# meiqua/6DPose

Hardware: AMD Instinct MI355X
Metric: templates*Mpixels matched/sec on 640x480 RGB-D (higher is better)
Workload: dtype u8

## Files before the change

6dpose_amd/csrc/detector.cpp:

```cpp
#include <math.h>
#include <stdarg.h>
#include <stdio.h>
#include <stdlib.h>
#include <string.h>

#include <algorithm>
#include <system_error>
#include <chrono>
#include <memory>
#include <string>
#include <vector>
#include <map>

#include "detector_internal.h"
#include <sched.h>
#include <ctype.h>
#include "render_internal.h"

static thread_local std::string g_err;
int lm_set_error(int code, const char* fmt, ...) {
    char buf[1024];
    va_list ap;
    va_start(ap, fmt);
    vsnprintf(buf, sizeof(buf), fmt, ap);
// ... 147 lines not shown
    if (d->mstream) (void)hipStreamSynchronize(d->mstream);
    d->frame_rgb.release(); d->frame_depth.release(); d->nrm_raw.release();
    for (int i = 0; i < lm_detector::kSlots; ++i) {
        if (d->ingest.pinned[i]) (void)hipHostFree(d->ingest.pinned[i]);
        d->ingest.d_rgb[i].release();
        if (d->ingest.t0[i]) (void)hipEventDestroy(d->ingest.t0[i]);
        if (d->ingest.t1[i]) (void)hipEventDestroy(d->ingest.t1[i]);
    }
    if (d->ingest.stream) (void)hipStreamDestroy(d->ingest.stream);
    for (int a = 0; a < lm_detector::kSlots; ++a) { d->lm_arena[a].release(); d->sm_arena[a].release(); }
    for (int a = 0; a < lm_detector::kSlots; ++a) { d->bits_arena[a].release(); d->cbits_arena[a].release(); }
    for (auto& b : d->slot_rgb) b.release();
    for (auto& b : d->slot_depth) b.release();
    for (auto& l : d->lvl) { l.rgb.release(); l.mag.release(); l.ang.release(); l.nrm.release(); l.mask[0].release(); l.mask[1].release(); }
    d->d_entries.release(); d->d_feat_off.release(); d->d_feat_xy.release(); d->d_feat_word.release(); d->d_run_mask.release(); d->d_work.release();
    d->d_cands.release(); d->d_counters.release(); d->d_final.release(); d->d_matches_dev.release(); d->d_hash.release(); d->d_distinct_keys.release(); d->d_tiles.release(); d->d_todo.release(); d->d_work_cls.release(); d->d_work_tid.release();
    for (int l = 0; l < kMaxLevels; ++l) { d->train.mask[l].release(); d->train.lab[l].release(); d->train.hrun[l].release(); }
    d->train.user_mask.release();
    d->train.keys.release(); d->train.counts.release(); d->train.bbox.release(); d->train.out.release();
    for (auto& sl : d->slot) {
        if (sl.h_matches) (void)hipHostFree(sl.h_matches);
        if (sl.h_distinct) (void)hipHostFree(sl.h_distinct);
        if (sl.h_counters) (void)hipHostFree(sl.h_counters);
        if (sl.fe_done) (void)hipEventDestroy(sl.fe_done);
        for (auto& e : sl.ev) if (e) (void)hipEventDestroy(e);
        if (sl.done) (void)hipEventDestroy(sl.done);
    }
    if (d->xchg.stream) (void)hipStreamSynchronize(d->xchg.stream);
    for (int a = 0; a < lm_detector::kSlots; ++a) {
        d->xchg.d_merged[a].release();
        d->xchg.d_runs.release();
// ... 1174 lines not shown
}
static bool cbits_active(const lm_detector* d, int num_work) {
    return bits_active(d, num_work) && knobs().coarse_bits && d->coarse_mode == 0 && d->cbits_max_nf <= 16383;
}
static int frame_slot(lm_detector* d, int si, bool tiled, uint32_t tile_cap, FrameSlot* out) {
    lm_detector::Slot& sl = d->slot[si];
    const uint32_t cc = d->buf_cand_cap;
    FrameSlot F{};
    F.lm_arena = d->lm_arena[si].p; F.sm_arena = d->sm_arena[si].p;
    F.cands = d->d_cands.p + (size_t)cc * si;
    F.tiles = tiled ? d->d_tiles.p + (size_t)tile_cap * si : nullptr;
    F.todo = tiled ? d->d_todo.p + (size_t)cc * si : nullptr;
    F.counters = d->d_counters.p + (size_t)kCounterWords * si;
    F.matches_dev = d->d_matches_dev.p + (size_t)cc * si;
    F.dedupe_table = d->d_hash.p + dedupe_table_slots(cc) * (size_t)si;
    F.distinct_keys = d->d_distinct_keys.p + (size_t)cc * si;
    F.final_dev = d->d_final.p + 8 * (size_t)si;
    F.matches = nullptr;
    HIP_TRY(hipHostGetDevicePointer((void**)&F.distinct, sl.h_distinct, 0));
    HIP_TRY(hipHostGetDevicePointer((void**)&F.final_host, sl.h_counters, 0));
    *out = F;
    return LM_OK;
}

static int slot_begin(lm_detector* d, float threshold, const char* const* class_ids, int num_class_ids, const uint8_t* rgb, const uint16_t* depth,
                      const bool have_mask[2], int ring) {
    if (d->n_submitted - d->n_collected >= (uint64_t)lm_detector::kSlots)
        return lm_set_error(LM_ERR_INVALID, "%d frames already in flight: call lm_detector_collect first", lm_detector::kSlots);
    HIP_TRY(hipSetDevice(d->device));
    int rc;
// ... 6 lines not shown
        if (class_ids && num_class_ids > 0)
            for (int i = 0; i < num_class_ids; ++i) key.push_back(class_ids[i] ? class_ids[i] : "");
        const bool same = d->work_valid && key == d->work_key && d->work_key_rank == d->shard_rank && d->work_key_world == d->shard_world;
        if (d->pend_n && (!same || threshold != d->pend_threshold) && (rc = lm_launch_pending(d))) return rc;
    }
    if ((rc = build_work(d, class_ids, num_class_ids))) return rc;
    const int num_work = (int)d->work_pyr.size();
    const int K = lm_detector::kSlots;
    if (d->buf_cand_cap < d->cand_cap) {
        if ((rc = lm_launch_pending(d))) return rc;
        if ((rc = sync_all_streams(d))) return rc;
        const uint32_t cc = d->cand_cap;
        if ((rc = d->d_cands.ensure((size_t)cc * K))) return rc;
        if ((rc = d->d_matches_dev.ensure((size_t)cc * K))) return rc;
        if ((rc = d->d_hash.ensure(dedupe_table_slots(cc) * K))) return rc;
        if ((rc = d->d_distinct_keys.ensure((size_t)cc * K))) return rc;
        d->buf_cand_cap = cc;
    }
    if (!d->d_counters.p) {
        if ((rc = d->d_counters.ensure((size_t)kCounterWords * K))) return rc;
        if ((rc = d->d_final.ensure(8 * (size_t)K))) return rc;
        HIP_TRY(hipMemset(d->d_counters.p, 0, (size_t)kCounterWords * K * sizeof(unsigned long long)));
        HIP_TRY(hipMemset(d->d_final.p, 0, 8 * (size_t)K * sizeof(unsigned long long)));
    }
    const bool tiled = (tiles_wanted(d) && num_work > 0 && tile_plan_possible(d->geom)) || bits_active(d, num_work);
    const uint32_t tile_cap = d->buf_cand_cap / 2;
    if (tiled && (d->d_tiles.cap < (size_t)tile_cap * K || d->d_todo.cap < (size_t)d->buf_cand_cap * K)) {
        if ((rc = lm_launch_pending(d))) return rc;
        if ((rc = sync_all_streams(d))) return rc;
        if ((rc = d->d_tiles.ensure((size_t)tile_cap * K))) return rc;
// ... 72 lines not shown
    FrameBatch fb{};
    fb.nb = nb;
    int rc;
    for (int b = 0; b < nb; ++b)
        if ((rc = frame_slot(d, (first + b) % lm_detector::kSlots, tiled, tile_cap, &fb.f[b]))) return rc;
    hipStream_t ms = d->mstream, s = ms;
    for (int b = nb - 1; b >= 0; --b) {
        const int ring = d->slot[(first + b) % lm_detector::kSlots].ring;
        if (ring < 0) continue;
        if (hipEventQuery(d->ingest.t1[ring]) != hipSuccess) { (void)hipGetLastError(); HIP_TRY(hipStreamWaitEvent(s, d->ingest.t1[ring], 0)); }
        break;
    }
    if ((rc = order_after_default_stream(d, s))) return rc;
    HIP_TRY(hipEventRecord(lead.ev[0], s));
    const bool cbits = cbits_active(d, num_work);
    bool direct_low = knobs().fe_bits && d->fe_direct && bits && d->bits_all_in, direct_top = knobs().fe_bits && d->fe_direct && cbits;
    for (int l = 0; l + 1 < d->geom.levels; ++l) direct_low = direct_low && fe_bits_rows_possible(d->geom.lv[l].W, d->geom.lv[l].T);
    const LevelGeom& topl = d->geom.lv[d->geom.levels - 1];
    const uint32_t top_bit0[2] = {topl.lm_off[0] - d->cbits_byte0, topl.lm_off[1] - d->cbits_byte0};
    const bool top_ored = direct_top && fe_top_bits_kind(topl.W, topl.H, topl.T, top_bit0, d->fe_top_mode) == kFeTopBits;
    if (top_ored)
        for (int b = 0; b < nb; ++b) {
            const int si = (first + b) % lm_detector::kSlots;
            if (!d->cbits_clean[si]) HIP_TRY(hipMemsetAsync(d->cbits_arena[si].p, 0, (size_t)d->cbits_npairs * 8, s));
            d->cbits_clean[si] = false;
        }
#ifdef LM_DIAG
    static double lp_t[6]; static long lp_n;
    auto lp_now = [] { return std::chrono::duration<double>(std::chrono::steady_clock::now().time_since_epoch()).count(); };
    const double lp0 = host_seconds(tp_launch0), lp1 = lp_now();
// ... 28 lines not shown
    bool resident_in = false;
    for (int b = 0; b < nb; ++b) resident_in = resident_in || d->slot[(first + b) % lm_detector::kSlots].ring < 0;
    HIP_TRY(hipEventRecord(lead.ev[1], s));
    if (resident_in) HIP_TRY(hipEventRecord(lead.fe_done, s));
    for (int b = 0; b < nb; ++b)
        if (d->slot[(first + b) % lm_detector::kSlots].ring < 0) d->resident_reader = lead.fe_done;
    for (int b = 0; b < nb; ++b) {
        const lm_detector::Slot& sl = d->slot[(first + b) % lm_detector::kSlots];
        if (sl.ring < 0 && d->ingest.stream)
            for (int r = 0; r < lm_detector::kSlots; ++r)
                if (d->ingest.d_rgb[r].p && sl.in_rgb == d->ingest.d_rgb[r].p) d->ingest.reader[r] = lead.fe_done;
    }
    const uint32_t cap = std::min<uint32_t>(lead.match_cap, d->buf_cand_cap);
    auto enqueue_coarse = [&](hipStream_t st) -> int {
        { LM_CLOCK("launch_coarse");
        if (cbits) launch_coarse_bits(fb, tb, d->geom, d->d_entries.p, d->d_feat_off.p, d->d_work.p, num_work, threshold, d->buf_cand_cap, d->cbits_byte0, d->cbits_max_nf, st);
        else launch_coarse(fb, d->geom, d->d_entries.p, d->d_feat_off.p, d->d_work.p, num_work, threshold, d->buf_cand_cap, tile_cap, st);
        }
        HIP_TRY(hipEventRecord(lead.ev[3], st));
        return LM_OK;
    };
    auto enqueue_match = [&]() -> int {
        if (bits) {
            { LM_CLOCK("launch_local_bits");
            launch_local_bits(fb, bb, d->geom, d->d_entries.p, d->d_feat_word.p, d->d_work.p, d->buf_cand_cap, threshold, cap,
                              (uint32_t)dedupe_table_slots(d->buf_cand_cap), bits_grid(d, nb), d->bits_max_nf, ms); }
            if (bb.top_clear_units)
                for (int b = 0; b < nb; ++b)
                    if (bb.top_clear[b]) d->cbits_clean[(first + b) % lm_detector::kSlots] = true;
            if (!d->bits_all_in)
                launch_local(fb_rest, d->geom, d->d_entries.p, d->d_feat_off.p, d->d_feat_word.p, d->d_run_mask.p, d->d_feat_xy.p, d->d_work.p, d->buf_cand_cap, threshold, cap,
                             (uint32_t)dedupe_table_slots(d->buf_cand_cap), tile_cap, d->num_cus * 2, ms);
        } else
        if (num_work > 0)
            launch_local(fb, d->geom, d->d_entries.p, d->d_feat_off.p, d->d_feat_word.p, d->d_run_mask.p, d->d_feat_xy.p, d->d_work.p, d->buf_cand_cap, threshold, cap,
                         (uint32_t)dedupe_table_slots(d->buf_cand_cap), tile_cap, local_grid(d, nb), ms);
        HIP_TRY(hipEventRecord(lead.ev[4], ms));
        return LM_OK;
    };
    const int dedupe_blocks = knobs().dedupe_blocks > 0 ? knobs().dedupe_blocks
                                                        : std::max(64, std::min(d->num_cus * 2, (int)((d->ncand_hint + 255) / 256)));
    auto enqueue_dedupe = [&](hipStream_t st) -> int {
        if (num_work > 0) {
            LM_CLOCK("launch_dedupe");
            launch_dedupe(fb, d->buf_cand_cap, dedupe_table_slots(d->buf_cand_cap), d->d_work_cls.p, d->d_work_tid.p, dedupe_blocks, st);
        }
        else
            for (int b = 0; b < nb; ++b) HIP_TRY(hipMemsetAsync(fb.f[b].final_dev, 0, 8 * sizeof(unsigned long long), st));
        return LM_OK;
    };
    {
#ifdef LM_DIAG
        const double lp3 = lp_now();
#endif
        if ((rc = enqueue_coarse(ms))) return rc;
#ifdef LM_DIAG
        const double lp4 = lp_now();
// ... 293 lines not shown
    lm_timings tm{};
    tm.h2d_ms = sl.h2d_ms; tm.templates = sl.num_work; tm.coarse_bytes = sl.coarse_bytes;
    if (d->ingest.used[slot_index]) {
        d->ingest.used[slot_index] = false;
        float h = 0.f;
        if (hipEventElapsedTime(&h, d->ingest.t0[slot_index], d->ingest.t1[slot_index]) == hipSuccess) tm.h2d_ms = h;
    }
    const uint64_t evals = sl.num_work > 0 ? hc[5] : 0, lbytes = sl.num_work > 0 ? hc[6] : 0;
    uint64_t nm = 0;
    const Candidate* hm = sl.h_matches;
    if (sl.num_work > 0 && ncand > 0 && (sort_unique == 0 || sort_unique == 3 || d->reference_order))
        HIP_TRY(hipMemcpy(sl.h_matches, sl.matches_dev, (size_t)ncand * sizeof(Candidate), hipMemcpyDeviceToHost));
    if (sl.num_work == 0) nm = 0;
    else if (sort_unique == 0) { for (uint64_t i = 0; i < ncand; ++i) nm += hm[i].work >= 0; }
    else nm = hc[2];
    tm.coarse_candidates = (int64_t)ncand;
    d->ncand_hint = (uint64_t)ncand;
    tm.local_evals = (int64_t)evals;
    tm.local_bytes = (int64_t)lbytes;
    tm.matches_pre_unique = (int64_t)nm;
    tm.d2h_ms = 0.f;
    tm.batch_frames = sl.batch_n;
    if (hipEventElapsedTime(&tm.frontend_ms, lead.ev[0], lead.ev[1]) != hipSuccess ||
        hipEventElapsedTime(&tm.coarse_ms, lead.ev[1], lead.ev[3]) != hipSuccess ||
        hipEventElapsedTime(&tm.local_ms, lead.ev[3], lead.ev[4]) != hipSuccess ||
        hipEventElapsedTime(&tm.total_ms, lead.ev[0], lead.ev[4]) != hipSuccess) {
        (void)hipGetLastError();
        tm.frontend_ms = tm.coarse_ms = tm.local_ms = tm.d2h_ms = tm.total_ms = 0.f;
    }
    if (sort_unique < 0) {
// ... 231 lines not shown
    d->fe_direct = on != 0;
    d->fe_keep_top = (on & 2) != 0;
    d->fe_top_mode = (on & 4) ? 1 : ((on & 8) ? 2 : 0);
    return LM_OK;
}

extern "C" int lm_detector_get_paths(const lm_detector* d, int* refine, int* coarse) {
    if (!d || !refine || !coarse) return lm_set_error(LM_ERR_INVALID, "null argument");
    if (d->bank_dirty) return lm_set_error(LM_ERR_INVALID, "no match yet: the paths follow from the bank and the frame geometry");
    const bool bits = bits_active(d, 1);
    *refine = bits ? 0 : (d->geom.levels >= 2 && tiles_wanted(d) && tile_plan_possible(d->geom) ? 1 : 2);
    *coarse = cbits_active(d, 1) ? 0 : 1;
    return LM_OK;
}

extern "C" int lm_detector_flush(lm_detector* d) {
    if (!d) return lm_set_error(LM_ERR_INVALID, "null detector");
    return lm_launch_pending(d);
}

extern "C" int lm_detector_set_batch(lm_detector* d, int frames) {
    if (!d) return lm_set_error(LM_ERR_INVALID, "null detector");
    if (frames < 1 || frames > kMaxBatch) return lm_set_error(LM_ERR_INVALID, "frames per launch must be in [1, %d]", kMaxBatch);
    int rc = lm_launch_pending(d);
    if (rc) return rc;
    d->batch_max = frames;
    return LM_OK;
}

extern "C" int lm_detector_get_batch(const lm_detector* d) { return d ? d->batch_max : 0; }
// ... 98 lines not shown
```

6dpose_amd/csrc/detector_internal.h:

```cpp
#pragma once
#include <atomic>
#include <chrono>
#include <condition_variable>
#include <deque>
#include <functional>
#include <memory>
#include <mutex>
#include <string>
#include <thread>
#include <vector>

#include "../../include/amd_linemod.h"
#include "host_templates.h"
#include "knobs.h"
#include "lm_kernels.h"

int lm_set_error(int code, const char* fmt, ...);

#define HIP_TRY(expr)                                                                                         \
    do {                                                                                                      \
        hipError_t _e = (expr);                                                                               \
        if (_e != hipSuccess) return lm_set_error(LM_ERR_HIP, "%s failed: %s (%s:%d)", #expr, hipGetErrorString(_e), \
                                                  __FILE__, __LINE__);                                        \
    } while (0)
// ... 72 lines not shown
    std::vector<TemplEntry> h_entries;
    DevBuf<TemplEntry> d_entries;
    DevBuf<int32_t> d_feat_off;
    DevBuf<uint32_t> d_feat_xy;
    DevBuf<uint32_t> d_feat_word, d_run_mask;
    std::vector<int32_t> work_pyr;
    std::shared_ptr<std::vector<int32_t>> work_cls, work_tid;
    DevBuf<int32_t> d_work;
    std::vector<std::string> work_key;
    int work_key_rank = -1, work_key_world = -1;
    bool work_valid = false;
    int64_t work_coarse_bytes = 0;
    DevBuf<Candidate> d_cands;
    DevBuf<Candidate> d_matches_dev;
    DevBuf<unsigned long long> d_hash;
    DevBuf<TileRec> d_tiles;
    DevBuf<uint8_t> d_todo;
    bool use_tiles = true;
    bool reference_order = false;
    DevBuf<ulonglong2> d_distinct_keys;
    DevBuf<int32_t> d_work_cls, d_work_tid;
    DevBuf<unsigned long long> d_counters;
    DevBuf<unsigned long long> d_final;
    uint32_t cand_cap = 1u << 18;
    uint32_t buf_cand_cap = 0;
    struct Slot {
        Candidate* h_matches = nullptr;
        Candidate* h_distinct = nullptr;
        uint32_t match_cap = 0;
        unsigned long long* h_counters = nullptr;
// ... 130 lines not shown
```

6dpose_amd/csrc/knobs.h:

```cpp
#pragma once
#include <stdlib.h>

#ifndef LM_FE_WAVES
#define LM_FE_WAVES 7
#endif
constexpr int kFeWaves = LM_FE_WAVES;

namespace lm {

struct Knobs {
    int coarse_group = 4;
    int local_blocks = 0;
    int frame_batch = 0;
    int coarse_bits = 1;
    int bitplanes = 1;
    int fe_bits = 1;
    int fe_bits_split = 0;
    int first_batch = 3;
    int fe_rows_cs = 0;
    int nt_copy = 1;
    int dedupe_blocks = 0;
    int fe_wgs_per_cu = kFeWaves;
    int launch_slack_us = 0;
    int batch_queue = 0;
    int knn_blocks = 0;
    int icp_splits = 0;
    int icp_team = 0;
    int icp_builds = 0;
    int icp_team_min_points = 128;
    int icp_cut_index = 3;
    int icp_relaunch = 1;
    int icp_wide_sort = 1;
    int icp_maxshift = 3;
    int icp_maxshift_late = 4;
#ifdef LM_DIAG
    int coarse_dbg = 0;
// ... 6 lines not shown
    static const Knobs k = [] {
        Knobs v;
        auto geti = [](const char* name, int dflt) { const char* e = getenv(name); return e && e[0] ? atoi(e) : dflt; };
        v.coarse_group = geti("LM_COARSE_GROUP", v.coarse_group);
        v.local_blocks = geti("LM_LOCAL_BLOCKS", 0);
        v.frame_batch = geti("LM_FRAME_BATCH", 0);
        v.batch_queue = geti("LM_BATCH_QUEUE", 0);
        v.launch_slack_us = geti("LM_LAUNCH_SLACK_US", 0);
        v.fe_wgs_per_cu = geti("LM_FE_WGS_PER_CU", kFeWaves);
        v.bitplanes = geti("LM_BITPLANES", 1);
        v.coarse_bits = geti("LM_COARSE_BITS", 1);
        v.fe_bits = geti("LM_FE_BITS", 1);
        v.fe_bits_split = geti("LM_FE_BITS_SPLIT", 0);
        v.first_batch = geti("LM_FIRST_BATCH", v.first_batch);
        v.dedupe_blocks = geti("LM_DEDUPE_BLOCKS", 0);
        v.nt_copy = geti("LM_NT_COPY", 1);
        v.fe_rows_cs = geti("LM_FE_ROWS_CS", 0);
        v.knn_blocks = geti("LM_KNN_BLOCKS", 0);
        v.icp_splits = geti("LM_ICP_SPLITS", 0);
        v.icp_team = geti("LM_ICP_TEAM", 0);
        v.icp_builds = geti("LM_ICP_BUILDS", 0);
        v.icp_wide_sort = geti("LM_ICP_WIDE_SORT", 1);
        v.icp_relaunch = geti("LM_ICP_RELAUNCH", 1);
        v.icp_cut_index = geti("LM_ICP_CUT_INDEX", 3);
        v.icp_team_min_points = geti("LM_ICP_TEAM_MIN_POINTS", 128);
        if (v.icp_team_min_points < 1) v.icp_team_min_points = 1;
        v.icp_maxshift = geti("LM_ICP_MAXSHIFT", v.icp_maxshift);
        v.icp_maxshift_late = geti("LM_ICP_MAXSHIFT_LATE", v.icp_maxshift_late);
#ifdef LM_DIAG
        v.coarse_dbg = geti("LM_COARSE_DBG", 0);
// ... 10 lines not shown
```

6dpose_amd/csrc/lm_kernels.h:

```cpp
#pragma once
#include <hip/hip_runtime.h>
#include <stdint.h>

namespace lm {

void upload_normal_lut(const uint8_t lut400[400]);
void launch_color_quant(const uint8_t* rgb, float* mag, uint8_t* onehot, int W, int H, float thr_sq, hipStream_t s);
void launch_normals_fused(const uint16_t* depth, uint8_t* raw, uint8_t* med, int W, int H, int dist_thr, int diff_thr, hipStream_t s);
void launch_pyrdown_rgb(const uint8_t* src, uint8_t* dst, int W, int H, hipStream_t s);
void launch_nn_down2(const uint8_t* src, uint8_t* dst, int W, int H, hipStream_t s);
void launch_build_lm(const uint8_t* const quant[2], const uint8_t* const mask[2], uint8_t* const lm[2], uint8_t* const strips[2],
                     int W, int H, int T, hipStream_t s);

struct LmJob { const uint8_t* quant; const uint8_t* mask; uint8_t* lm; uint8_t* strips; };
enum { kFeNone = 0, kFeColour, kFeNormals, kFePyrDown, kFeNnDown, kFeBuildLm, kFeBitsRows, kFeTopBits, kFeTopBitsAligned, kFeTopBitsTile, kFeBitsRowsTile };
struct FeJob {
    int kind, gx, gy, gz, first;
    const void* in; void* out0; void* out1;
    int W, H, a, b;
    float f;
    uint32_t m_gx, m_gxgy, m_wd, m_t, m_np;
    int Wd, Hd;
    LmJob lm[2];
};
// ... 51 lines not shown
constexpr int kCandBits = 40;
constexpr unsigned long long kCandMask = (1ull << kCandBits) - 1ull;
constexpr int kMaxBatch = 8;
constexpr int kCounterWords = 64;
constexpr int kStatShards = 16;
struct FrameSlot {
    const uint8_t* lm_arena;
    const uint8_t* sm_arena;
    Candidate* cands;
    TileRec* tiles;
    uint8_t* todo;
    unsigned long long* counters;
    Candidate* matches;
    Candidate* matches_dev;
    unsigned long long* dedupe_table;
    Candidate* distinct;
    ulonglong2* distinct_keys;
    unsigned long long* final_dev;
    unsigned long long* final_host;
};
struct FrameBatch {
    int nb;
    int pad;
    FrameSlot f[kMaxBatch];
};

struct BitsBatch { const uint8_t* strips[kMaxBatch]; uint8_t* bits[kMaxBatch];
                   uint8_t* top_clear[kMaxBatch]; uint32_t top_clear_units; };
constexpr int kBitsSmallMax = 511;
void launch_pack_bits(const BitsBatch& B, int nb, const LevelGeom& lv, hipStream_t s);
void launch_local_bits(const FrameBatch& fb, const BitsBatch& B, const FrameGeom& g, const TemplEntry* entries, const uint32_t* feat_word,
                       const int32_t* work_pyramids, uint32_t cand_cap, float threshold, uint32_t cap, uint32_t dedupe_cap_slots, int grid_blocks,
                       int max_features, hipStream_t s);
struct TopBits { const uint8_t* lm[kMaxBatch]; uint8_t* bits[kMaxBatch]; };
void launch_pack_top(const TopBits& B, int nb, uint32_t byte0, uint32_t npairs, hipStream_t s);
void launch_coarse_bits(const FrameBatch& fb, const TopBits& B, const FrameGeom& g, const TemplEntry* entries, const int32_t* feat_off,
                        const int32_t* work_pyramids, int num_work, float threshold, uint32_t cap, uint32_t byte0, int max_features, hipStream_t s);
bool tile_plan_possible(const FrameGeom& g);
size_t coarse_plan_lds_bytes(int Wd, int Hd);
void launch_coarse(const FrameBatch& fb, const FrameGeom& g, const TemplEntry* entries, const int32_t* feat_off,
                   const int32_t* work_pyramids, int num_work, float threshold, uint32_t cap, uint32_t tile_cap, hipStream_t s);
constexpr int kRunMax = 62;
void launch_local(const FrameBatch& fb, const FrameGeom& g, const TemplEntry* entries, const int32_t* feat_off, const uint32_t* feat_word,
                  const uint32_t* run_mask, const uint32_t* feat_xy, const int32_t* work_pyramids, uint32_t cand_cap, float threshold, uint32_t cap,
                  uint32_t dedupe_cap_slots, uint32_t tile_cap, int grid_blocks, hipStream_t s);
__host__ __device__ inline uint32_t dedupe_slots_for(uint32_t n, uint32_t cap_slots) {
    uint32_t t = 1024;
    while (t < 2u * n && t < cap_slots) t <<= 1;
    return t < cap_slots ? t : cap_slots;
}

struct TopkSel {
// ... 56 lines not shown
```

6dpose_amd/csrc/match.hip:

```cpp
#include <algorithm>

#include "knobs.h"
#include "lm_kernels.h"

namespace lm {

static __device__ __forceinline__ uint32_t ld_u32(const uint8_t* p) {
    uint32_t v;
    __builtin_memcpy(&v, p, 4);
    return v;
}

static __device__ __forceinline__ float score_of(int raw, int nfeat) {
    return __fdiv_rn(__fmul_rn((float)raw, 100.f), (float)(4 * nfeat));
}


using BufRsrc = __amdgpu_buffer_rsrc_t;
static __device__ __forceinline__ BufRsrc make_rsrc(const void* base) {
    return __builtin_amdgcn_make_buffer_rsrc(const_cast<void*>(base), 0, -1 , 0x00020000 );
}
static __device__ __forceinline__ uint4 ld_buf16(BufRsrc r, uint32_t lane_off, uint32_t uniform_off) {
    const auto v = __builtin_amdgcn_raw_buffer_load_b128(r, (int)lane_off, (int)uniform_off, 0);
    uint4 u;
// ... 789 lines not shown
__global__ void __launch_bounds__(256)
k_pack_bits(BitsBatch B, uint32_t sm_off0, uint32_t records, int NS, int Hd) {
    const uint32_t i = blockIdx.x * 256u + threadIdx.x;
    if (i >= records) return;
    const uint32_t q = i / (uint32_t)Hd, s = q % (uint32_t)NS;
    const uint8_t* src = B.strips[blockIdx.y] + sm_off0 + (size_t)i * 16;
    const uint4 a = *reinterpret_cast<const uint4*>(src);
    uint4 b = make_uint4(0, 0, 0, 0);
    if (s + 1 < (uint32_t)NS) b = *reinterpret_cast<const uint4*>(src + (size_t)Hd * 16);
    uint2 r;
    r.x = pack16(a);
    r.y = pack16(b);
    *reinterpret_cast<uint2*>(B.bits[blockIdx.y] + (sm_off0 >> 1) + (size_t)i * 8) = r;
}

template <int kHi, int kWaves>
__global__ void __launch_bounds__(256) __attribute__((amdgpu_waves_per_eu(kWaves, kWaves)))
k_local_bits(FrameBatch fb, BitsBatch B, FrameGeom g, const TemplEntry* __restrict__ entries, const uint32_t* __restrict__ feat_word,
             const int32_t* __restrict__ work_pyramids, uint32_t cand_cap, float threshold, uint32_t cap, uint32_t dedupe_cap_slots) {
    constexpr int kN = 4 + kHi;
    constexpr int kS = kN + 3;
    __shared__ unsigned long long s_acc[kMaxBatch][2];
    __shared__ uint32_t s_cnt[kMaxBatch];
    const int lane = threadIdx.x & 63, grp = lane >> 3, j = lane & 7;
    const int nb = fb.nb;
    int f_lo = 0, f_hi = nb;
    uint32_t w_first = blockIdx.x * (blockDim.x >> 6) + (threadIdx.x >> 6), w_step = gridDim.x * (blockDim.x >> 6);
    if (nb > 1 && nb <= 8 && (gridDim.x & 7) == 0) {
        const int xcd = (int)(blockIdx.x & 7);
        f_lo = xcd % nb; f_hi = f_lo + 1;
        const uint32_t mine = (uint32_t)((7 - f_lo) / nb + 1);
        const uint32_t wpb = blockDim.x >> 6;
        w_first = ((blockIdx.x >> 3) * mine + (uint32_t)(xcd / nb)) * wpb + (threadIdx.x >> 6);
        w_step = (gridDim.x >> 3) * mine * wpb;
    }
    if ((int)threadIdx.x < nb) {
        const unsigned long long nc = fb.f[threadIdx.x].counters[0] & kCandMask;
        s_cnt[threadIdx.x] = nc < cand_cap ? (uint32_t)nc : cand_cap;
        s_acc[threadIdx.x][0] = 0; s_acc[threadIdx.x][1] = 0;
    }
    __syncthreads();
    for (int f = 0; f < nb; ++f) {
        unsigned long long* table = fb.f[f].dedupe_table;
        if (!table) continue;
        const uint32_t tsize = dedupe_slots_for(s_cnt[f], dedupe_cap_slots);
        for (uint32_t i = blockIdx.x * blockDim.x + threadIdx.x; i < tsize; i += gridDim.x * blockDim.x) table[i] = ~0ull;
    }
    if (B.top_clear_units)
        for (int f = 0; f < nb; ++f)
            for (uint32_t i = blockIdx.x * blockDim.x + threadIdx.x; i < B.top_clear_units; i += gridDim.x * blockDim.x)
                reinterpret_cast<uint4*>(B.top_clear[f])[i] = make_uint4(0u, 0u, 0u, 0u);
    const int src0 = (lane & ~7) << 2;
    const uint32_t rowoff = 16u * (uint32_t)j;
    for (int fr = f_lo; fr < f_hi; ++fr) {
        const FrameSlot& F = fb.f[fr];
        const BufRsrc bits = make_rsrc(B.bits[fr]);
        const uint32_t nc = s_cnt[fr], ngroups = (nc + 7u) >> 3;
        for (uint32_t gi = w_first; gi < ngroups; gi += w_step) {
            const uint32_t ci = gi * 8u + (uint32_t)grp;
            const bool valid = ci < nc;
            Candidate cd{0, 0, 0.f, 0};
            if (valid) cd = F.cands[ci];
            const int work = cd.work;
            const int pyr = work_pyramids[work];
            int mx = cd.x, my = cd.y;
            float sim = cd.score;
            bool alive = valid, leave = false;
            uint32_t evals = 0, bytes = 0;
            for (int l = g.levels - 2; l >= 0; --l) {
                const LevelGeom& lv = g.lv[l];
                const int T = lv.T, W = lv.W, H = lv.H, Wd = lv.Wd, Hd = lv.Hd;
                const int border = 8 * T, offset = T / 2 + (T % 2 - 1);
// ... 104 lines not shown
                float best = 0.f;
                if (raw > 0) {
                    const int idx = 255 - (int)(key & 0xFF);
                    br = idx >> 4; bc = idx & 15;
                    best = score_of(raw, nf);
                }
                if (run) {
                    ++evals;
                    bytes += 256u * (uint32_t)nf;
                    sim = best;
                    mx = (x / T - 8 + bc) * T + offset;
                    my = (y / T - 8 + br) * T + offset;
                    if (sim < threshold) alive = false;
                }
            }
            if (valid && j == 0) {
                F.todo[ci] = leave ? 1 : 0;
                if (!leave) {
                    if (ci < cap) {
                        Candidate m;
                        m.x = mx; m.y = my; m.score = sim;
                        m.work = alive ? work : -1;
                        F.matches_dev[ci] = m;
                    }
                    atomicAdd(&s_acc[fr][0], (unsigned long long)evals);
                    atomicAdd(&s_acc[fr][1], (unsigned long long)bytes);
                }
            }
        }
    }
    __syncthreads();
    if ((int)threadIdx.x < nb && s_acc[threadIdx.x][0] != 0) {
        unsigned long long* st = fb.f[threadIdx.x].counters + 8 + 2 * (blockIdx.x & (kStatShards - 1));
        atomicAdd(st, s_acc[threadIdx.x][0]);
        atomicAdd(st + 1, s_acc[threadIdx.x][1]);
    }
}

void launch_pack_bits(const BitsBatch& B, int nb, const LevelGeom& lv, hipStream_t s) {
    const uint32_t records = (uint32_t)(2 * 8 * lv.T * lv.T) * (uint32_t)lv.NS * (uint32_t)lv.Hd;
    hipLaunchKernelGGL(k_pack_bits, dim3((records + 255) / 256, nb), dim3(256), 0, s, B, lv.sm_off[0], records, lv.NS, lv.Hd);
}
void launch_local_bits(const FrameBatch& fb, const BitsBatch& B, const FrameGeom& g, const TemplEntry* entries, const uint32_t* feat_word,
                       const int32_t* work_pyramids, uint32_t cand_cap, float threshold, uint32_t cap, uint32_t dedupe_cap_slots, int grid_blocks,
                       int max_features, hipStream_t s) {
    if (max_features > kBitsSmallMax)
        hipLaunchKernelGGL((k_local_bits<10, 4>), dim3(grid_blocks), dim3(256), 0, s, fb, B, g, entries, feat_word, work_pyramids, cand_cap, threshold, cap, dedupe_cap_slots);
    else
        hipLaunchKernelGGL((k_local_bits<5, 4>), dim3(grid_blocks), dim3(256), 0, s, fb, B, g, entries, feat_word, work_pyramids, cand_cap, threshold, cap, dedupe_cap_slots);
}

__global__ void __launch_bounds__(256)
k_pack_top(TopBits B, uint32_t byte0, uint32_t npairs) {
    const uint32_t i = blockIdx.x * 256u + threadIdx.x;
    if (i >= npairs) return;
    const uint8_t* src = B.lm[blockIdx.y] + byte0 + (size_t)i * 32;
    const uint4 a = *reinterpret_cast<const uint4*>(src), b = *reinterpret_cast<const uint4*>(src + 16);
    auto four = [](uint32_t d, int sh) -> uint32_t { return ((((d >> sh) & 0x01010101u) * 0x01020408u) >> 24) & 0xFu; };
    auto bits = [&](const uint4& v, int sh) -> uint32_t { return four(v.x, sh) | (four(v.y, sh) << 4) | (four(v.z, sh) << 8) | (four(v.w, sh) << 12); };
    uint2 r;
    r.x = bits(a, 0) | (bits(b, 0) << 16);
    r.y = bits(a, 2) | (bits(b, 2) << 16);
    *reinterpret_cast<uint2*>(B.bits[blockIdx.y] + (size_t)i * 8) = r;
}

template <int kHi, int kWaves>
__global__ void __launch_bounds__(256) __attribute__((amdgpu_waves_per_eu(kWaves, kWaves)))
k_coarse_bits(FrameBatch fb, TopBits B, LevelGeom lv, int level, int levels, const TemplEntry* __restrict__ entries, const int32_t* __restrict__ feat_off,
              const int32_t* __restrict__ work_pyramids, int num_work, float threshold, uint32_t cap, uint32_t byte0) {
    constexpr int kN = 4 + kHi, kS = kN + 3;
    __shared__ uint32_t s_tot[4];
    __shared__ unsigned long long s_base;
    const FrameSlot& F = fb.f[blockIdx.y];
    Candidate* __restrict__ cands = F.cands;
    unsigned long long* __restrict__ counters = F.counters;
    const int lane = threadIdx.x & 63;
    const int wave = __builtin_amdgcn_readfirstlane((int)(threadIdx.x >> 6));
    const int work_raw = (int)blockIdx.x * 4 + wave;
    const bool live = work_raw < num_work;
    const int work = live ? work_raw : num_work - 1;
    const int pyr = work_pyramids[work];
    const TemplEntry e = entries[(size_t)pyr * levels + level];
    const int nf = e.nf, nfp = e.nf_padded;
    const int32_t* fo = feat_off + e.feat_start;
    const int Wd = lv.Wd, Hd = lv.Hd, T = lv.T, npos = Wd * Hd;
    const int wf = (e.width - 1) / T + 1, hf = (e.height - 1) / T + 1;
    const int tp = (Hd - hf) * Wd + (Wd - wf) + 1;
    const int offset = T / 2 + (T % 2 - 1);
// ... 87 lines not shown
                    const int cy = jpos / Wd, cx = jpos - cy * Wd;
                    Candidate c;
                    c.x = cx * T + offset; c.y = cy * T + offset; c.score = score_of(raw, nf); c.work = work;
                    cands[slot] = c;
                }
                ++slot;
            }
        }
    }
}

void launch_pack_top(const TopBits& B, int nb, uint32_t byte0, uint32_t npairs, hipStream_t s) {
    hipLaunchKernelGGL(k_pack_top, dim3((npairs + 255) / 256, nb), dim3(256), 0, s, B, byte0, npairs);
}
void launch_coarse_bits(const FrameBatch& fb, const TopBits& B, const FrameGeom& g, const TemplEntry* entries, const int32_t* feat_off,
                        const int32_t* work_pyramids, int num_work, float threshold, uint32_t cap, uint32_t byte0, int max_features, hipStream_t s) {
    if (num_work <= 0 || fb.nb <= 0) return;
    const int level = g.levels - 1;
#define LM_LAUNCH_COARSE_BITS(HI, WAVES) \
    hipLaunchKernelGGL((k_coarse_bits<HI, WAVES>), dim3((num_work + 3) / 4, fb.nb), dim3(256), 0, s, fb, B, g.lv[level], level, g.levels, entries, feat_off, \
                       work_pyramids, num_work, threshold, cap, byte0)
    if (max_features > kBitsSmallMax) LM_LAUNCH_COARSE_BITS(10, 5);
    else LM_LAUNCH_COARSE_BITS(5, 6);
#undef LM_LAUNCH_COARSE_BITS
}

void launch_local(const FrameBatch& fb, const FrameGeom& g, const TemplEntry* entries, const int32_t* feat_off, const uint32_t* feat_word,
                  const uint32_t* run_mask, const uint32_t* feat_xy, const int32_t* work_pyramids, uint32_t cand_cap, float threshold, uint32_t cap,
                  uint32_t dedupe_cap_slots, uint32_t tile_cap, int grid_blocks, hipStream_t s) {
    if (grid_blocks <= 0 || fb.nb <= 0) return;
    int dbg = 0;
#ifdef LM_DIAG
    dbg = knobs().local_dbg;
#endif
    hipLaunchKernelGGL(k_local, dim3(grid_blocks), dim3(256), 0, s, fb, g, entries, feat_off, feat_word, run_mask, feat_xy, work_pyramids, cand_cap,
                       threshold, cap, dedupe_cap_slots, tile_cap, dbg);
// ... 4 lines not shown
```

6dpose_amd/linemodLevelup_pybind.py:

```python
from __future__ import annotations

import ctypes
import gzip
import os
import sys
import shutil
import tempfile
from typing import List, Optional, Sequence

import numpy as np

__all__ = ["Detector", "Match", "poseRefine", "IcpContext", "Pipeline", "Mesh", "Template", "library_path", "load_library", "nms",
           "pose_errors", "gt_stats"]

_HERE = os.path.dirname(os.path.abspath(__file__))
_LIB_NAME = "libamdlinemod.so"
_lib = None


class _CMatch(ctypes.Structure):
    _fields_ = [("x", ctypes.c_int32), ("y", ctypes.c_int32), ("similarity", ctypes.c_float),
                ("class_index", ctypes.c_int32), ("template_id", ctypes.c_int32)]


# ... 482 lines not shown
        f.restype = ctypes.c_int
        _check(f(self._h, self._REFINE[refine], self._COARSE[coarse]))
        g = self._lib.lm_detector_set_direct_bits
        g.argtypes = [ctypes.c_void_p, ctypes.c_int]
        g.restype = ctypes.c_int
        _check(g(self._h, int(direct)))

    def getPaths(self):
        f = self._lib.lm_detector_get_paths
        f.argtypes = [ctypes.c_void_p, ctypes.POINTER(ctypes.c_int), ctypes.POINTER(ctypes.c_int)]
        f.restype = ctypes.c_int
        r, c = ctypes.c_int(), ctypes.c_int()
        _check(f(self._h, ctypes.byref(r), ctypes.byref(c)))
        return ({v: k for k, v in self._REFINE.items()}[r.value], {v: k for k, v in self._COARSE.items()}[c.value])

    def getBatch(self) -> int:
        return int(self._lib.lm_detector_get_batch(self._h))

    def ingestBuffers(self, width: int, height: int):
        pr, pd = ctypes.c_void_p(), ctypes.c_void_p()
        _check(self._lib.lm_detector_ingest_buffer(self._h, int(width), int(height), ctypes.byref(pr), ctypes.byref(pd)))
        n = int(width) * int(height)
        rgb = np.ctypeslib.as_array(ctypes.cast(pr, ctypes.POINTER(ctypes.c_uint8)), shape=(n * 3,)).reshape(height, width, 3)
        depth = np.ctypeslib.as_array(ctypes.cast(pd, ctypes.POINTER(ctypes.c_uint16)), shape=(n,)).reshape(height, width)
        return rgb, depth

    def matchStream(self, frames, threshold: float, class_ids: Sequence[str] = (), depth: int = 3):
        depth = max(1, min(int(depth), self._lib.lm_detector_max_in_flight()))
        pending = []

# ... 514 lines not shown
```

include/amd_linemod.h:

```cpp
#ifndef AMD_LINEMOD_H
#define AMD_LINEMOD_H

#include <stddef.h>
#include <stdint.h>

#ifdef __cplusplus
extern "C" {
#endif

#define LM_OK 0
#define LM_ERR_INVALID (-2)
#define LM_ERR_NO_DEVICE (-3)
#define LM_ERR_HIP (-4)
#define LM_ERR_IO (-5)
#define LM_ERR_NOT_FOUND (-6)
#define LM_ERR_OVERFLOW (-7)

typedef struct lm_detector lm_detector;

typedef struct lm_match {
    int32_t x;
    int32_t y;
    float similarity;
    int32_t class_index;
// ... 98 lines not shown
int lm_detector_submit(lm_detector *d, float threshold, const char *const *class_ids, int num_class_ids);
int lm_detector_collect(lm_detector *d, int sort_unique, lm_match **out, size_t *n);
int lm_detector_set_reference_order(lm_detector *d, int on);
int lm_detector_submit_frame(lm_detector *d, const uint8_t *rgb, const uint16_t *depth, int width, int height,
                             float threshold, const char *const *class_ids, int num_class_ids);
int lm_detector_ingest_buffer(lm_detector *d, int width, int height, uint8_t **rgb, uint16_t **depth);
int lm_detector_flush(lm_detector *d);
int lm_detector_set_batch(lm_detector *d, int frames);
int lm_detector_get_batch(const lm_detector *d);
int lm_detector_set_batch_queue(lm_detector *d, int batches);
int lm_detector_set_async_collect(lm_detector *d, int on);
int lm_detector_host_profile(lm_detector *d, double *out8, int reset);
int lm_detector_refines_on_bit_planes(const lm_detector *d);
int lm_detector_set_paths(lm_detector *d, int refine, int coarse);
int lm_detector_get_paths(const lm_detector *d, int *refine, int *coarse);
int lm_detector_set_direct_bits(lm_detector *d, int on);
int lm_detector_last_timings(const lm_detector *d, lm_timings *t);

int64_t lm_detector_read_stage(lm_detector *d, int level, int kind, uint8_t *dst, int64_t capacity);

size_t lm_merge_matches(lm_match *m, size_t n);

int lm_nms_boxes(const double *boxes, const double *scores, int n, double thresh, int32_t *keep);
int lm_nms_norms(const double *ts, const double *scores, int n, double thresh, int32_t *keep);
int lm_nms_boxes_cv(const int32_t *rects, const float *scores, int n, float score_threshold, float nms_threshold, float eta,
                    int top_k, int32_t *keep);

void lm_free(void *p);

#define LM_ICP_SCENE_FROM_SCENE 1
// ... 90 lines not shown
```

Measured before the change: 10.42 million.

## Fuse candidate dedupe into local bit-plane refine kernel with dirty-slot hash cleanup

When the bit-plane coarse and refine paths are both active, the separate dedupe kernel is skipped. Survivors are instead inserted into the hash table and compacted into the distinct list inside k_local_bits, and the last block to finish writes the final counters. Instead of clearing the whole hash table every frame, the coarse kernel of the next frame resets only the slots recorded in a dirty list. This removes a kernel launch and a full table clear per frame, at the cost of extra atomics and a cross-block completion counter in the refine kernel.

```diff
diff --git a/6dpose_amd/csrc/detector.cpp b/6dpose_amd/csrc/detector.cpp
--- a/6dpose_amd/csrc/detector.cpp
+++ b/6dpose_amd/csrc/detector.cpp
@@ -185,7 +185,7 @@
     for (auto& b : d->slot_depth) b.release();
     for (auto& l : d->lvl) { l.rgb.release(); l.mag.release(); l.ang.release(); l.nrm.release(); l.mask[0].release(); l.mask[1].release(); }
     d->d_entries.release(); d->d_feat_off.release(); d->d_feat_xy.release(); d->d_feat_word.release(); d->d_run_mask.release(); d->d_work.release();
-    d->d_cands.release(); d->d_counters.release(); d->d_final.release(); d->d_matches_dev.release(); d->d_hash.release(); d->d_distinct_keys.release(); d->d_tiles.release(); d->d_todo.release(); d->d_work_cls.release(); d->d_work_tid.release();
+    d->d_cands.release(); d->d_counters.release(); d->d_final.release(); d->d_matches_dev.release(); d->d_hash.release(); d->d_dirty.release(); d->d_distinct_keys.release(); d->d_tiles.release(); d->d_todo.release(); d->d_work_cls.release(); d->d_work_tid.release();
     for (int l = 0; l < kMaxLevels; ++l) { d->train.mask[l].release(); d->train.lab[l].release(); d->train.hrun[l].release(); }
     d->train.user_mask.release();
     d->train.keys.release(); d->train.counts.release(); d->train.bbox.release(); d->train.out.release();
@@ -1390,6 +1390,7 @@
     F.counters = d->d_counters.p + (size_t)kCounterWords * si;
     F.matches_dev = d->d_matches_dev.p + (size_t)cc * si;
     F.dedupe_table = d->d_hash.p + dedupe_table_slots(cc) * (size_t)si;
+    F.dirty = d->d_dirty.p + (size_t)cc * si;
     F.distinct_keys = d->d_distinct_keys.p + (size_t)cc * si;
     F.final_dev = d->d_final.p + 8 * (size_t)si;
     F.matches = nullptr;
@@ -1426,6 +1427,8 @@
         if ((rc = d->d_cands.ensure((size_t)cc * K))) return rc;
         if ((rc = d->d_matches_dev.ensure((size_t)cc * K))) return rc;
         if ((rc = d->d_hash.ensure(dedupe_table_slots(cc) * K))) return rc;
+        if ((rc = d->d_dirty.ensure((size_t)cc * K))) return rc;
+        for (int k = 0; k < K; ++k) d->hash_listed[k] = false;
         if ((rc = d->d_distinct_keys.ensure((size_t)cc * K))) return rc;
         d->buf_cand_cap = cc;
     }
@@ -1528,6 +1531,16 @@
     if ((rc = order_after_default_stream(d, s))) return rc;
     HIP_TRY(hipEventRecord(lead.ev[0], s));
     const bool cbits = cbits_active(d, num_work);
+    const bool fused = bits && cbits && d->bits_all_in && knobs().fuse_dedupe;
+    d->last_dedupe_fused = fused;
+    for (int b = 0; b < nb; ++b) {
+        const int si = (first + b) % lm_detector::kSlots;
+        if (fused && !d->hash_listed[si]) {
+            HIP_TRY(hipMemsetAsync(fb.f[b].dedupe_table, 0xFF, dedupe_table_slots(d->buf_cand_cap) * sizeof(unsigned long long), s));
+            HIP_TRY(hipMemsetAsync(fb.f[b].final_dev + kFinalDirty, 0, sizeof(unsigned long long), s));
+        }
+        d->hash_listed[si] = fused;
+    }
     bool direct_low = knobs().fe_bits && d->fe_direct && bits && d->bits_all_in, direct_top = knobs().fe_bits && d->fe_direct && cbits;
     for (int l = 0; l + 1 < d->geom.levels; ++l) direct_low = direct_low && fe_bits_rows_possible(d->geom.lv[l].W, d->geom.lv[l].T);
     const LevelGeom& topl = d->geom.lv[d->geom.levels - 1];
@@ -1586,7 +1599,8 @@
     const uint32_t cap = std::min<uint32_t>(lead.match_cap, d->buf_cand_cap);
     auto enqueue_coarse = [&](hipStream_t st) -> int {
         { LM_CLOCK("launch_coarse");
-        if (cbits) launch_coarse_bits(fb, tb, d->geom, d->d_entries.p, d->d_feat_off.p, d->d_work.p, num_work, threshold, d->buf_cand_cap, d->cbits_byte0, d->cbits_max_nf, st);
+        if (cbits) launch_coarse_bits(fb, tb, d->geom, d->d_entries.p, d->d_feat_off.p, d->d_work.p, num_work, threshold, d->buf_cand_cap, d->cbits_byte0, d->cbits_max_nf,
+                                      fused ? (uint32_t)dedupe_table_slots(d->buf_cand_cap) : 0u, st);
         else launch_coarse(fb, d->geom, d->d_entries.p, d->d_feat_off.p, d->d_work.p, num_work, threshold, d->buf_cand_cap, tile_cap, st);
         }
         HIP_TRY(hipEventRecord(lead.ev[3], st));
@@ -1596,7 +1610,7 @@
         if (bits) {
             { LM_CLOCK("launch_local_bits");
             launch_local_bits(fb, bb, d->geom, d->d_entries.p, d->d_feat_word.p, d->d_work.p, d->buf_cand_cap, threshold, cap,
-                              (uint32_t)dedupe_table_slots(d->buf_cand_cap), bits_grid(d, nb), d->bits_max_nf, ms); }
+                              (uint32_t)dedupe_table_slots(d->buf_cand_cap), bits_grid(d, nb), d->bits_max_nf, fused ? d->d_work_cls.p : nullptr, d->d_work_tid.p, ms); }
             if (bb.top_clear_units)
                 for (int b = 0; b < nb; ++b)
                     if (bb.top_clear[b]) d->cbits_clean[(first + b) % lm_detector::kSlots] = true;
@@ -1613,6 +1627,7 @@
     const int dedupe_blocks = knobs().dedupe_blocks > 0 ? knobs().dedupe_blocks
                                                         : std::max(64, std::min(d->num_cus * 2, (int)((d->ncand_hint + 255) / 256)));
     auto enqueue_dedupe = [&](hipStream_t st) -> int {
+        if (fused) return LM_OK;
         if (num_work > 0) {
             LM_CLOCK("launch_dedupe");
             launch_dedupe(fb, d->buf_cand_cap, dedupe_table_slots(d->buf_cand_cap), d->d_work_cls.p, d->d_work_tid.p, dedupe_blocks, st);
@@ -1936,6 +1951,7 @@
     if (sl.num_work == 0) nm = 0;
     else if (sort_unique == 0) { for (uint64_t i = 0; i < ncand; ++i) nm += hm[i].work >= 0; }
     else nm = hc[2];
+    d->last_distinct = sl.num_work > 0 ? (int64_t)hc[1] : 0;
     tm.coarse_candidates = (int64_t)ncand;
     d->ncand_hint = (uint64_t)ncand;
     tm.local_evals = (int64_t)evals;
@@ -2197,6 +2213,13 @@
     return LM_OK;
 }
 
+extern "C" int lm_detector_get_fusion(const lm_detector* d, int* dedupe_fused, int64_t* last_distinct) {
+    if (!d || !dedupe_fused) return lm_set_error(LM_ERR_INVALID, "null argument");
+    *dedupe_fused = d->last_dedupe_fused ? 1 : 0;
+    if (last_distinct) *last_distinct = d->last_distinct;
+    return LM_OK;
+}
+
 extern "C" int lm_detector_flush(lm_detector* d) {
     if (!d) return lm_set_error(LM_ERR_INVALID, "null detector");
     return lm_launch_pending(d);
diff --git a/6dpose_amd/csrc/detector_internal.h b/6dpose_amd/csrc/detector_internal.h
--- a/6dpose_amd/csrc/detector_internal.h
+++ b/6dpose_amd/csrc/detector_internal.h
@@ -110,6 +110,10 @@
     DevBuf<Candidate> d_cands;
     DevBuf<Candidate> d_matches_dev;
     DevBuf<unsigned long long> d_hash;
+    DevBuf<uint32_t> d_dirty;
+    bool hash_listed[kSlots] = {};
+    int64_t last_distinct = 0;
+    bool last_dedupe_fused = false;
     DevBuf<TileRec> d_tiles;
     DevBuf<uint8_t> d_todo;
     bool use_tiles = true;
diff --git a/6dpose_amd/csrc/knobs.h b/6dpose_amd/csrc/knobs.h
--- a/6dpose_amd/csrc/knobs.h
+++ b/6dpose_amd/csrc/knobs.h
@@ -20,6 +20,7 @@
     int fe_rows_cs = 0;
     int nt_copy = 1;
     int dedupe_blocks = 0;
+    int fuse_dedupe = 1;
     int fe_wgs_per_cu = kFeWaves;
     int launch_slack_us = 0;
     int batch_queue = 0;
@@ -56,6 +57,7 @@
         v.fe_bits_split = geti("LM_FE_BITS_SPLIT", 0);
         v.first_batch = geti("LM_FIRST_BATCH", v.first_batch);
         v.dedupe_blocks = geti("LM_DEDUPE_BLOCKS", 0);
+        v.fuse_dedupe = geti("LM_FUSE_DEDUPE", 1);
         v.nt_copy = geti("LM_NT_COPY", 1);
         v.fe_rows_cs = geti("LM_FE_ROWS_CS", 0);
         v.knn_blocks = geti("LM_KNN_BLOCKS", 0);
diff --git a/6dpose_amd/csrc/lm_kernels.h b/6dpose_amd/csrc/lm_kernels.h
--- a/6dpose_amd/csrc/lm_kernels.h
+++ b/6dpose_amd/csrc/lm_kernels.h
@@ -89,11 +89,13 @@
     Candidate* matches;
     Candidate* matches_dev;
     unsigned long long* dedupe_table;
+    uint32_t* dirty;
     Candidate* distinct;
     ulonglong2* distinct_keys;
     unsigned long long* final_dev;
     unsigned long long* final_host;
 };
+constexpr int kFinalDirty = 7;
 struct FrameBatch {
     int nb;
     int pad;
@@ -106,11 +108,12 @@
 void launch_pack_bits(const BitsBatch& B, int nb, const LevelGeom& lv, hipStream_t s);
 void launch_local_bits(const FrameBatch& fb, const BitsBatch& B, const FrameGeom& g, const TemplEntry* entries, const uint32_t* feat_word,
                        const int32_t* work_pyramids, uint32_t cand_cap, float threshold, uint32_t cap, uint32_t dedupe_cap_slots, int grid_blocks,
-                       int max_features, hipStream_t s);
+                       int max_features, const int32_t* work_cls, const int32_t* work_tid, hipStream_t s);
 struct TopBits { const uint8_t* lm[kMaxBatch]; uint8_t* bits[kMaxBatch]; };
 void launch_pack_top(const TopBits& B, int nb, uint32_t byte0, uint32_t npairs, hipStream_t s);
 void launch_coarse_bits(const FrameBatch& fb, const TopBits& B, const FrameGeom& g, const TemplEntry* entries, const int32_t* feat_off,
-                        const int32_t* work_pyramids, int num_work, float threshold, uint32_t cap, uint32_t byte0, int max_features, hipStream_t s);
+                        const int32_t* work_pyramids, int num_work, float threshold, uint32_t cap, uint32_t byte0, int max_features,
+                        uint32_t clean_slots, hipStream_t s);
 bool tile_plan_possible(const FrameGeom& g);
 size_t coarse_plan_lds_bytes(int Wd, int Hd);
 void launch_coarse(const FrameBatch& fb, const FrameGeom& g, const TemplEntry* entries, const int32_t* feat_off,
diff --git a/6dpose_amd/csrc/match.hip b/6dpose_amd/csrc/match.hip
--- a/6dpose_amd/csrc/match.hip
+++ b/6dpose_amd/csrc/match.hip
@@ -827,13 +827,14 @@
     *reinterpret_cast<uint2*>(B.bits[blockIdx.y] + (sm_off0 >> 1) + (size_t)i * 8) = r;
 }
 
-template <int kHi, int kWaves>
+template <int kHi, int kWaves, bool kFused>
 __global__ void __launch_bounds__(256) __attribute__((amdgpu_waves_per_eu(kWaves, kWaves)))
 k_local_bits(FrameBatch fb, BitsBatch B, FrameGeom g, const TemplEntry* __restrict__ entries, const uint32_t* __restrict__ feat_word,
-             const int32_t* __restrict__ work_pyramids, uint32_t cand_cap, float threshold, uint32_t cap, uint32_t dedupe_cap_slots) {
+             const int32_t* __restrict__ work_pyramids, uint32_t cand_cap, float threshold, uint32_t cap, uint32_t dedupe_cap_slots,
+             const int32_t* __restrict__ work_cls, const int32_t* __restrict__ work_tid) {
     constexpr int kN = 4 + kHi;
     constexpr int kS = kN + 3;
-    __shared__ unsigned long long s_acc[kMaxBatch][2];
+    __shared__ unsigned long long s_acc[kMaxBatch][3];
     __shared__ uint32_t s_cnt[kMaxBatch];
     const int lane = threadIdx.x & 63, grp = lane >> 3, j = lane & 7;
     const int nb = fb.nb;
@@ -850,10 +851,10 @@
     if ((int)threadIdx.x < nb) {
         const unsigned long long nc = fb.f[threadIdx.x].counters[0] & kCandMask;
         s_cnt[threadIdx.x] = nc < cand_cap ? (uint32_t)nc : cand_cap;
-        s_acc[threadIdx.x][0] = 0; s_acc[threadIdx.x][1] = 0;
+        s_acc[threadIdx.x][0] = 0; s_acc[threadIdx.x][1] = 0; s_acc[threadIdx.x][2] = 0;
     }
     __syncthreads();
-    for (int f = 0; f < nb; ++f) {
+    for (int f = 0; f < nb && !kFused; ++f) {
         unsigned long long* table = fb.f[f].dedupe_table;
         if (!table) continue;
         const uint32_t tsize = dedupe_slots_for(s_cnt[f], dedupe_cap_slots);
@@ -869,6 +870,7 @@
         const FrameSlot& F = fb.f[fr];
         const BufRsrc bits = make_rsrc(B.bits[fr]);
         const uint32_t nc = s_cnt[fr], ngroups = (nc + 7u) >> 3;
+        const uint32_t table_mask = dedupe_slots_for(nc, dedupe_cap_slots) - 1u;
         for (uint32_t gi = w_first; gi < ngroups; gi += w_step) {
             const uint32_t ci = gi * 8u + (uint32_t)grp;
             const bool valid = ci < nc;
@@ -1003,26 +1005,88 @@
                     if (sim < threshold) alive = false;
                 }
             }
+            Candidate m{0, 0, 0.f, -1};
+            bool rec_alive = false, keep = false;
+            uint32_t claimed = ~0u;
             if (valid && j == 0) {
                 F.todo[ci] = leave ? 1 : 0;
                 if (!leave) {
                     if (ci < cap) {
-                        Candidate m;
                         m.x = mx; m.y = my; m.score = sim;
                         m.work = alive ? work : -1;
                         F.matches_dev[ci] = m;
+                        if (kFused && alive) {
+                            rec_alive = true;
+                            const bool packable = mx >= -32768 && mx <= 32767 && my >= -32768 && my <= 32767;
+                            keep = !packable;
+                            if (packable) {
+                                const unsigned long long key = ((unsigned long long)(uint32_t)work << 32) | ((uint32_t)(mx & 0xFFFF) << 16) | (uint32_t)(my & 0xFFFF);
+                                const unsigned long long hsh = key * 0x9E3779B97F4A7C15ull;
+                                uint32_t slot = (uint32_t)(hsh >> 40) & table_mask;
+                                for (;;) {
+                                    const unsigned long long prev = atomicCAS(&F.dedupe_table[slot], ~0ull, key);
+                                    if (prev == ~0ull) { keep = true; claimed = slot; break; }
+                                    if (prev == key) break;
+                                    slot = (slot + 1) & table_mask;
+                                }
+                            }
+                        }
                     }
                     atomicAdd(&s_acc[fr][0], (unsigned long long)evals);
                     atomicAdd(&s_acc[fr][1], (unsigned long long)bytes);
                 }
             }
+            if (kFused) {
+                const unsigned long long mk = __ballot(keep), ma = __ballot(rec_alive);
+                if (ma) {
+                    unsigned long long base = 0;
+                    if (lane == 0) {
+                        if (mk) base = atomicAdd(&F.counters[1], (unsigned long long)__popcll(mk));
+                        atomicAdd(&s_acc[fr][2], (unsigned long long)__popcll(ma));
+                    }
+                    base = bcast_u64(base, 0);
+                    if (keep) {
+                        const unsigned long long at = base + __popcll(mk & ((1ull << lane) - 1ull));
+                        F.distinct[at] = m;
+                        F.dirty[at] = claimed;
+                        if (F.distinct_keys) {
+                            const int cls = work_cls[work], tid = work_tid[work];
+                            F.distinct_keys[at] = xchg_make_key(m.x, m.y, m.score, cls, tid);
+                            if (!xchg_key_fits(m.x, m.y, cls, tid)) atomicOr(&F.counters[3], 1ull);
+                        }
+                    }
+                }
+            }
         }
     }
     __syncthreads();
-    if ((int)threadIdx.x < nb && s_acc[threadIdx.x][0] != 0) {
+    if ((int)threadIdx.x < nb && (s_acc[threadIdx.x][0] != 0 || s_acc[threadIdx.x][2] != 0)) {
         unsigned long long* st = fb.f[threadIdx.x].counters + 8 + 2 * (blockIdx.x & (kStatShards - 1));
-        atomicAdd(st, s_acc[threadIdx.x][0]);
-        atomicAdd(st + 1, s_acc[threadIdx.x][1]);
+        if (s_acc[threadIdx.x][0] != 0) { atomicAdd(st, s_acc[threadIdx.x][0]); atomicAdd(st + 1, s_acc[threadIdx.x][1]); }
+        if (kFused && s_acc[threadIdx.x][2] != 0) atomicAdd(&fb.f[threadIdx.x].counters[2], s_acc[threadIdx.x][2]);
+    }
+    if (kFused) {
+        asm volatile("s_waitcnt vmcnt(0)" ::: "memory");
+        __syncthreads();
+        const int f = (int)threadIdx.x;
+        if (f >= f_lo && f < f_hi) {
+            const FrameSlot& F = fb.f[f];
+            unsigned long long* __restrict__ counters = F.counters;
+            const bool by_xcd = nb > 1 && f_hi - f_lo == 1;
+            const unsigned long long serving = by_xcd ? (unsigned long long)(gridDim.x >> 3) * (unsigned long long)((7 - f) / nb + 1) : (unsigned long long)gridDim.x;
+            if (atomicAdd(&counters[7], 1ull) == serving - 1ull) {
+                const unsigned long long c0 = atomicAdd(&counters[0], 0ull), nc = c0 & kCandMask;
+                const unsigned long long nd = atomicAdd(&counters[1], 0ull), na = atomicAdd(&counters[2], 0ull), bad = atomicAdd(&counters[3], 0ull);
+                unsigned long long evals = 0, lbytes = 0;
+                for (int q = 0; q < kStatShards; ++q) { evals += atomicAdd(&counters[8 + 2 * q], 0ull); lbytes += atomicAdd(&counters[9 + 2 * q], 0ull); }
+                F.final_dev[0] = nc; F.final_dev[1] = nd; F.final_dev[2] = na; F.final_dev[3] = bad;
+                F.final_dev[kFinalDirty] = nd;
+                F.final_host[0] = nc; F.final_host[1] = nd; F.final_host[2] = na; F.final_host[3] = bad;
+                F.final_host[4] = c0 >> kCandBits;
+                F.final_host[5] = evals; F.final_host[6] = lbytes;
+                for (int q = 0; q < kCounterWords; ++q) counters[q] = 0;
+            }
+        }
     }
 }
 
@@ -1032,11 +1096,14 @@
 }
 void launch_local_bits(const FrameBatch& fb, const BitsBatch& B, const FrameGeom& g, const TemplEntry* entries, const uint32_t* feat_word,
                        const int32_t* work_pyramids, uint32_t cand_cap, float threshold, uint32_t cap, uint32_t dedupe_cap_slots, int grid_blocks,
-                       int max_features, hipStream_t s) {
-    if (max_features > kBitsSmallMax)
-        hipLaunchKernelGGL((k_local_bits<10, 4>), dim3(grid_blocks), dim3(256), 0, s, fb, B, g, entries, feat_word, work_pyramids, cand_cap, threshold, cap, dedupe_cap_slots);
-    else
-        hipLaunchKernelGGL((k_local_bits<5, 4>), dim3(grid_blocks), dim3(256), 0, s, fb, B, g, entries, feat_word, work_pyramids, cand_cap, threshold, cap, dedupe_cap_slots);
+                       int max_features, const int32_t* work_cls, const int32_t* work_tid, hipStream_t s) {
+#define LM_LAUNCH_LOCAL_BITS(HI, FUSED) \
+    hipLaunchKernelGGL((k_local_bits<HI, 4, FUSED>), dim3(grid_blocks), dim3(256), 0, s, fb, B, g, entries, feat_word, work_pyramids, cand_cap, threshold, cap, \
+                       dedupe_cap_slots, work_cls, work_tid)
+    const bool fused = work_cls != nullptr;
+    if (max_features > kBitsSmallMax) { if (fused) LM_LAUNCH_LOCAL_BITS(10, true); else LM_LAUNCH_LOCAL_BITS(10, false); }
+    else { if (fused) LM_LAUNCH_LOCAL_BITS(5, true); else LM_LAUNCH_LOCAL_BITS(5, false); }
+#undef LM_LAUNCH_LOCAL_BITS
 }
 
 __global__ void __launch_bounds__(256)
@@ -1056,11 +1123,19 @@
 template <int kHi, int kWaves>
 __global__ void __launch_bounds__(256) __attribute__((amdgpu_waves_per_eu(kWaves, kWaves)))
 k_coarse_bits(FrameBatch fb, TopBits B, LevelGeom lv, int level, int levels, const TemplEntry* __restrict__ entries, const int32_t* __restrict__ feat_off,
-              const int32_t* __restrict__ work_pyramids, int num_work, float threshold, uint32_t cap, uint32_t byte0) {
+              const int32_t* __restrict__ work_pyramids, int num_work, float threshold, uint32_t cap, uint32_t byte0, uint32_t clean_slots) {
     constexpr int kN = 4 + kHi, kS = kN + 3;
     __shared__ uint32_t s_tot[4];
     __shared__ unsigned long long s_base;
     const FrameSlot& F = fb.f[blockIdx.y];
+    if (clean_slots) {
+        const unsigned long long listed = F.final_dev[kFinalDirty];
+        const uint32_t n = listed < cap ? (uint32_t)listed : cap;
+        for (uint32_t i = blockIdx.x * 256u + threadIdx.x; i < n; i += gridDim.x * 256u) {
+            const uint32_t at = F.dirty[i];
+            if (at < clean_slots) F.dedupe_table[at] = ~0ull;
+        }
+    }
     Candidate* __restrict__ cands = F.cands;
     unsigned long long* __restrict__ counters = F.counters;
     const int lane = threadIdx.x & 63;
@@ -1178,12 +1253,13 @@
     hipLaunchKernelGGL(k_pack_top, dim3((npairs + 255) / 256, nb), dim3(256), 0, s, B, byte0, npairs);
 }
 void launch_coarse_bits(const FrameBatch& fb, const TopBits& B, const FrameGeom& g, const TemplEntry* entries, const int32_t* feat_off,
-                        const int32_t* work_pyramids, int num_work, float threshold, uint32_t cap, uint32_t byte0, int max_features, hipStream_t s) {
+                        const int32_t* work_pyramids, int num_work, float threshold, uint32_t cap, uint32_t byte0, int max_features,
+                        uint32_t clean_slots, hipStream_t s) {
     if (num_work <= 0 || fb.nb <= 0) return;
     const int level = g.levels - 1;
 #define LM_LAUNCH_COARSE_BITS(HI, WAVES) \
     hipLaunchKernelGGL((k_coarse_bits<HI, WAVES>), dim3((num_work + 3) / 4, fb.nb), dim3(256), 0, s, fb, B, g.lv[level], level, g.levels, entries, feat_off, \
-                       work_pyramids, num_work, threshold, cap, byte0)
+                       work_pyramids, num_work, threshold, cap, byte0, clean_slots)
     if (max_features > kBitsSmallMax) LM_LAUNCH_COARSE_BITS(10, 5);
     else LM_LAUNCH_COARSE_BITS(5, 6);
 #undef LM_LAUNCH_COARSE_BITS
diff --git a/6dpose_amd/linemodLevelup_pybind.py b/6dpose_amd/linemodLevelup_pybind.py
--- a/6dpose_amd/linemodLevelup_pybind.py
+++ b/6dpose_amd/linemodLevelup_pybind.py
@@ -520,6 +520,22 @@
         _check(f(self._h, ctypes.byref(r), ctypes.byref(c)))
         return ({v: k for k, v in self._REFINE.items()}[r.value], {v: k for k, v in self._COARSE.items()}[c.value])
 
+    def getFusion(self) -> dict:
+        f = self._lib.lm_detector_get_fusion
+        f.argtypes = [ctypes.c_void_p, ctypes.POINTER(ctypes.c_int), ctypes.POINTER(ctypes.c_int64)]
+        f.restype = ctypes.c_int
+        dd = ctypes.c_int()
+        _check(f(self._h, ctypes.byref(dd), None))
+        return {"dedupe": bool(dd.value)}
+
+    def lastDistinct(self) -> int:
+        f = self._lib.lm_detector_get_fusion
+        f.argtypes = [ctypes.c_void_p, ctypes.POINTER(ctypes.c_int), ctypes.POINTER(ctypes.c_int64)]
+        f.restype = ctypes.c_int
+        dd, n = ctypes.c_int(), ctypes.c_int64()
+        _check(f(self._h, ctypes.byref(dd), ctypes.byref(n)))
+        return int(n.value)
+
     def getBatch(self) -> int:
         return int(self._lib.lm_detector_get_batch(self._h))
 
diff --git a/include/amd_linemod.h b/include/amd_linemod.h
--- a/include/amd_linemod.h
+++ b/include/amd_linemod.h
@@ -136,6 +136,7 @@
 int lm_detector_refines_on_bit_planes(const lm_detector *d);
 int lm_detector_set_paths(lm_detector *d, int refine, int coarse);
 int lm_detector_get_paths(const lm_detector *d, int *refine, int *coarse);
+int lm_detector_get_fusion(const lm_detector *d, int *dedupe_fused, int64_t *last_distinct);
 int lm_detector_set_direct_bits(lm_detector *d, int on);
 int lm_detector_last_timings(const lm_detector *d, lm_timings *t);
 
```

Result: slower. 6.190 million (-40.6%).
